# cvlab-kaist/3DGAN-Inversion

Hardware: AMD Instinct MI355X
Metric: inversion-steps/sec (G fwd+bwd, 512^2 FFHQ EG3D) at 1/2/4/8 GPUs; final PSNR (higher is better)
Workload: dtype f32 (modulated convs: two-piece fp16 split, 3 products, range-normalised; other GEMMs bf16x6; fp32-equivalent); 1 GPU; C2: FFHQ 512^2 single-image latent inversion step (Phase A, w + 17 noise maps per image; G.synthesis fwd+bwd, 128^2 x 96-sample rendering, stub-LPIPS feature distance + noise regulariser, Adam); images_per_gpu=1, world_size=1, generator=ffhqrebalanced512-128-shaped, 30.66 M params, random-init (synthetic weights), parallelism=1 independent images, 1 per GPU; stat all-reduce only, launch=one HIP graph replay per step

## Files before the change

3dgan-inversion_amd/csrc/renderer.hip:

```cpp
#include "common.h"
#include "det.h"
#include "render_common.h"

namespace {

constexpr int FC = 32;
constexpr int HD = 64;
constexpr int CO = 32;
#ifndef RK_MAXT
#define RK_MAXT 192
#endif
constexpr int MAXT = RK_MAXT;

__device__ __forceinline__ float sigmoidf_(float x) { return __frcp_rn(1.f + __expf(-x)); }
__device__ __forceinline__ float softplusf_(float x) { return fmaxf(x, 0.f) + __logf(1.f + __expf(-fabsf(x))); }
__device__ __forceinline__ float sigmoid_acc(float x) { return 1.f / (1.f + expf(-x)); }
__device__ __forceinline__ float softplus_acc(float x) { return x > 20.f ? x : log1pf(expf(x)); }

struct PlaneUV { float u, v; };

__device__ __forceinline__ void plane_uv(int pl, float x, float y, float z, float& u, float& v) {
    if (pl == 0) { u = x; v = y; } else if (pl == 1) { u = x; v = z; } else { u = z; v = x; }
}

// ... 519 lines not shown
    float* E = red + r * 2 * D;
    float* GA = red + RPB * 2 * D + r * 2 * D;
    float* GWT = red + 2 * RPB * 2 * D + r * 4 * D;
    float* DL = GWT + 2 * D;
    if (has_c) E[rank_c] = e_c;
    if (has_f) E[rank_f] = e_f;
    __syncthreads();
    float xw[2] = {0.f, 0.f};
    if (live) {
        const float wsum = L.misc[0], dnum = L.misc[1];
        const float depth_raw = dnum / wsum;
        const float dmin = p.depth_minmax[0], dmax = p.depth_minmax[1];
        float gd = bp.d_depth ? bp.d_depth[rr] : 0.f;
        if (!(depth_raw >= dmin && depth_raw <= dmax)) gd = 0.f;
        const float gws = bp.d_wsum ? bp.d_wsum[rr] : 0.f;
        float grgb_sum = 0.f;
        if (p.white_back) for (int k = 0; k < CO; ++k) grgb_sum += grgb[k];
        int k = 0;
        for (int i = s; i < nI; i += D, ++k) {
            const float dmid = 0.5f * (L.sd[i] + L.sd[i + 1]);
            float gw = (E[i] + E[i + 1]) + gws - 2.f * grgb_sum;
            if (gd != 0.f) gw += gd * (dmid - depth_raw) / wsum;
            const float m = 0.5f * (L.ss[i] + L.ss[i + 1]) - 1.f;
            GWT[i] = gw * L.t[i];
            DL[i] = L.sd[i + 1] - L.sd[i];
            GA[i] = m > 20.f ? 1.f : (RK_FAST_ALPHA ? sigmoidf_(m) : sigmoid_acc(m));
            xw[k] = gw * L.w[i];
        }
    }
    __syncthreads();
    if (live) {
        int k = 0;
        for (int i = s; i < nI; i += D, ++k) E[i] = xw[k];
    }
    __syncthreads();
    if (scan_lane) suffix_scan_inplace(red + tid * 2 * D, nI, 2 * D, vec);
    __syncthreads();
    if (live) {
        for (int i = s; i < nI; i += D) {
            const float q = L.q[i];
            const float galpha = GWT[i] - E[i] / q;
            const float one_minus_alpha = q - 1e-10f;
            const float gsp = galpha * DL[i] * one_minus_alpha;
            GA[i] = gsp * GA[i];
        }
    }
    __syncthreads();

    if (bp.df_amax != nullptr && blockIdx.x == 0 && tid == 0) *bp.df_amax = 0.f;
    if (live && s < D) {
        float4* pr = reinterpret_cast<float4*>(bp.df_pos);
        pr[(rr * 2 + 0) * D + s] = has_c ? make_float4(ox + depth_c * dx, oy + depth_c * dy, oz + depth_c * dz, depth_c) : make_float4(NAN, 0, 0, 0);
        pr[(rr * 2 + 1) * D + s] = has_f ? make_float4(ox + depth_f * dx, oy + depth_f * dy, oz + depth_f * dz, depth_f) : make_float4(NAN, 0, 0, 0);
    }
    if (has_c) {
        const float a = 0.5f * ((rank_c > 0 ? L.w[rank_c - 1] : 0.f) + (rank_c < nI ? L.w[rank_c] : 0.f));
        const float gs = 0.5f * ((rank_c > 0 ? GA[rank_c - 1] : 0.f) + (rank_c < nI ? GA[rank_c] : 0.f));
        reinterpret_cast<float2*>(bp.ag_rows)[(rr * 2 + 0) * D + s] = make_float2(a, gs);
    }
    if (has_f) {
        const float a = 0.5f * ((rank_f > 0 ? L.w[rank_f - 1] : 0.f) + (rank_f < nI ? L.w[rank_f] : 0.f));
        const float gs = 0.5f * ((rank_f > 0 ? GA[rank_f - 1] : 0.f) + (rank_f < nI ? GA[rank_f] : 0.f));
        reinterpret_cast<float2*>(bp.ag_rows)[(rr * 2 + 1) * D + s] = make_float2(a, gs);
    }
}

__global__ void __launch_bounds__(256) render_coord_reduce_kernel(const float4* __restrict__ gc, float* __restrict__ d_o, float* __restrict__ d_d,
                                                                  int64_t nrays, int rows_per_ray) {
    const int64_t ray = (int64_t)blockIdx.x * blockDim.x + threadIdx.x;
    if (ray >= nrays) return;
    float o0 = 0.f, o1 = 0.f, o2 = 0.f, d0 = 0.f, d1 = 0.f, d2 = 0.f;
    const float4* g = gc + ray * rows_per_ray;
    for (int i = 0; i < rows_per_ray; ++i) {
        const float4 v = g[i];
        o0 += v.x; o1 += v.y; o2 += v.z;
        d0 += v.x * v.w; d1 += v.y * v.w; d2 += v.z * v.w;
    }
    if (d_o) { d_o[ray * 3] = o0; d_o[ray * 3 + 1] = o1; d_o[ray * 3 + 2] = o2; }
    if (d_d) { d_d[ray * 3] = d0; d_d[ray * 3 + 1] = d1; d_d[ray * 3 + 2] = d2; }
}

constexpr int TS = 15;

__device__ __forceinline__ bool plane_cell(const float4 pos, int pl, float cs, int Hp, int Wp, int& x0, int& y0, float& wx1, float& wy1) {
    float u, v;
    plane_uv(pl, pos.x * cs, pos.y * cs, pos.z * cs, u, v);
    float ix = ((u + 1.f) * Wp - 1.f) * 0.5f, iy = ((v + 1.f) * Hp - 1.f) * 0.5f;
    float fx0 = floorf(ix), fy0 = floorf(iy);
    wx1 = ix - fx0; wy1 = iy - fy0;
    if (!(fx0 >= -1.f && fx0 <= (float)(Wp - 1) && fy0 >= -1.f && fy0 <= (float)(Hp - 1))) return false;
    x0 = (int)fx0; y0 = (int)fy0;
    return true;
}

__device__ __forceinline__ int tile_of(int x0, int y0, int ntx, int nty) {
    int tx = (x0 < 0 ? 0 : x0) / TS, ty = (y0 < 0 ? 0 : y0) / TS;
    return (ty < nty ? ty : nty - 1) * ntx + (tx < ntx ? tx : ntx - 1);
}

constexpr int BIN_ITEMS = 16;
template <int PASS>
__global__ void __launch_bounds__(256) scatter_bin_kernel(const float4* __restrict__ pos, int64_t S, int64_t rows_per_image, float cs, int Hp, int Wp,
                                                          int ntx, int nty, int nb, int* __restrict__ counts, const int* __restrict__ offsets,
                                                          int* __restrict__ fill, int* __restrict__ ids) {
    extern __shared__ int hist[];
    for (int i = threadIdx.x; i < nb; i += 256) hist[i] = 0;
    __syncthreads();
    int bin[BIN_ITEMS], lrank[BIN_ITEMS], rowi[BIN_ITEMS];
    const int64_t base = (int64_t)blockIdx.x * 256 * BIN_ITEMS + threadIdx.x;
#pragma unroll
    for (int k = 0; k < BIN_ITEMS; ++k) {
        bin[k] = -1;
        const int64_t i = base + (int64_t)k * 256;
        if (i >= S * 3) continue;
        const int64_t row = i / 3;
        const int pl = (int)(i - row * 3);
        const float4 ps = pos[row];
        if (isnan(ps.x)) continue;
        int x0, y0; float wx1, wy1;
        if (!plane_cell(ps, pl, cs, Hp, Wp, x0, y0, wx1, wy1)) continue;
        const int n = (int)(row / rows_per_image);
        bin[k] = (n * 3 + pl) * (ntx * nty) + tile_of(x0, y0, ntx, nty);
        rowi[k] = (int)row;
        lrank[k] = atomicAdd(&hist[bin[k]], 1);
    }
    __syncthreads();
    if constexpr (PASS == 0) {
        for (int i = threadIdx.x; i < nb; i += 256) { int c = hist[i]; if (c) atomicAdd(counts + i, c); }
    } else {
        int* basep = hist + nb;
        for (int i = threadIdx.x; i < nb; i += 256) { int c = hist[i]; basep[i] = c ? offsets[i] + atomicAdd(fill + i, c) : 0; }
        __syncthreads();
#pragma unroll
        for (int k = 0; k < BIN_ITEMS; ++k)
            if (bin[k] >= 0) {
                if (PASS == 1) {
                    ids[basep[bin[k]] + lrank[k]] = rowi[k] << 2;
                } else {
                    const int ntile = ntx * nty, t = bin[k] % ntile, pl = (bin[k] / ntile) % 3;
                    int x0, y0; float wx1, wy1;
                    plane_cell(pos[rowi[k]], pl, cs, Hp, Wp, x0, y0, wx1, wy1);
                    const int lx = x0 - (t % ntx) * TS, ly = y0 - (t / ntx) * TS;
                    reinterpret_cast<float4*>(ids)[basep[bin[k]] + lrank[k]] =
                        make_float4(__int_as_float(rowi[k]), __int_as_float(((ly + 1) << 16) | (lx + 1)), wx1, wy1);
                }
            }
    }
}

constexpr int CHUNK = 4096;

__global__ void __launch_bounds__(1024) scatter_scan_kernel(const int* __restrict__ counts, int* __restrict__ offsets, int* __restrict__ chunk_offsets, int n) {
    __shared__ int part[1024], partc[1024];
    const int t = threadIdx.x;
    const int per = (n + 1023) / 1024;
    int sum = 0, sumc = 0;
    for (int k = 0; k < per; ++k) { int idx = t * per + k; if (idx < n) { int c = counts[idx]; sum += c; sumc += (c + CHUNK - 1) / CHUNK; } }
    part[t] = sum; partc[t] = sumc;
    __syncthreads();
    for (int off = 1; off < 1024; off <<= 1) {
        int v = t >= off ? part[t - off] : 0, vc = t >= off ? partc[t - off] : 0;
        __syncthreads();
        part[t] += v; partc[t] += vc;
        __syncthreads();
    }
    int run = part[t] - sum, runc = partc[t] - sumc;
    for (int k = 0; k < per; ++k) {
        int idx = t * per + k;
        if (idx < n) { int c = counts[idx]; offsets[idx] = run; if (chunk_offsets) chunk_offsets[idx] = runc; run += c; runc += (c + CHUNK - 1) / CHUNK; }
    }
// ... 214 lines not shown
    lds_barrier();
    issue_R(0); issue_M(2);
    asm volatile("s_waitcnt vmcnt(3)" ::: "memory");
    lds_barrier();
    issue_R(1);
    for (int b = 0; b < nbat; ++b) {
        asm volatile("s_waitcnt vmcnt(2)" ::: "memory");
        lds_barrier();
        issue_M(b + 3);
        issue_R(b + 2);
        const float4* meta = reinterpret_cast<const float4*>(sm + NRB * ROWB + (b % NMB) * RECB);
        const float* dfb = reinterpret_cast<const float*>(sm + (b % NRB) * ROWB);
        int* cn = cnt[b & 1];
        if (tid < TROWS) cnt[(b + 1) & 1][tid] = 0;
        if (tid < BATCH && beg + b * BATCH + tid < end) {
            const int k = __float_as_int(meta[tid].y) >> 16;
            lists[k * BATCH + lds_add_rtn((unsigned)(uintptr_t)&cn[k], 1)] = (unsigned short)tid;
        }
        lds_barrier();
#pragma unroll
        for (int l = 0; l < LPW; ++l) {
            const int li = wave * LPW + l;
            const int m = cn[li];
            const unsigned short* lst = lists + li * BATCH;
            for (int e = 0; e < m; e += 8) {
                int j[4];
                float4 mt[4];
                float g[4];
#pragma unroll
                for (int q = 0; q < 4; ++q) j[q] = lst[min(e + 2 * q + kk, BATCH - 1)] & (BATCH - 1);
#pragma unroll
                for (int q = 0; q < 4; ++q) { mt[q] = meta[j[q]]; g[q] = dfb[j[q] * FC + c]; }
#pragma unroll
                for (int q = 0; q < 4; ++q) {
                    const bool live = e + 2 * q + kk < m;
                    const int lx = (__float_as_int(mt[q].y) & 0xffff) - 1;
                    const float wx = mx == lx ? 1.f - mt[q].z : (mx == lx + 1 ? mt[q].z : 0.f);
                    const float wy = mhalf ? mt[q].w : 1.f - mt[q].w;
                    acc[l] = __builtin_amdgcn_mfma_f32_32x32x2f32(live ? wx * wy : 0.f, live ? g[q] : 0.f, acc[l], 0, 0, 0);
                }
            }
        }
    }
    asm volatile("s_waitcnt vmcnt(0)" ::: "memory");
    __syncthreads();
#pragma unroll
    for (int l = 0; l < LPW; ++l) {
        const int li = wave * LPW + l;
#pragma unroll
        for (int r = 0; r < 16; ++r) {
            const int m = (r & 3) + 8 * (r >> 2) + 4 * kk;
            if (m >= 16) tile[(li * TROWS + (m & 15)) * FC + c] = acc[l][r];
        }
    }
    __syncthreads();
#pragma unroll
    for (int l = 0; l < LPW; ++l) {
        const int li = wave * LPW + l;
        if (li >= 1) {
#pragma unroll
            for (int r = 0; r < 16; ++r) {
                const int m = (r & 3) + 8 * (r >> 2) + 4 * kk;
                if (m < 16) tile[((li - 1) * TROWS + m) * FC + c] += acc[l][r];
            }
        }
    }
    __syncthreads();
    for (int i = tid; i < TILE_FLOATS; i += NT) {
        const float v = tile[i];
        if (v != 0.f) {
            const int cell = i / FC, ch = i - cell * FC;
            const int yy = ty0 + cell / TROWS, xx = tx0 + cell % TROWS;
            if (yy < Hp && xx < Wp) eg3d_acc(d_planes + (int64_t)n * Hp * Wp * ldp + ((int64_t)yy * Wp + xx) * ldp + pl * FC + ch, v);
        }
    }
}

constexpr int BIN16_THREADS = 1024;
constexpr int BIN16_ITEMS = 18;

template <int PASS, int SL>
__global__ void __launch_bounds__(BIN16_THREADS) scatter_bin16_kernel(const float4* __restrict__ pos, int64_t S, float cs, int Hp, int Wp, int ntx, int nty,
                                                            int nb16, int* __restrict__ counts, const int* __restrict__ offsets, int* __restrict__ fill,
                                                            float4* __restrict__ recs, int ray_w, int rpr) {
    extern __shared__ int hist[];
    for (int i = threadIdx.x; i < nb16; i += BIN16_THREADS) hist[i] = 0;
    __syncthreads();
    int bin[BIN16_ITEMS], lrank[BIN16_ITEMS], rowi[BIN16_ITEMS];
    const int ntile = ntx * nty;
    int brick_row0 = 0;
    if (SL > 0) {
        const int nslab = rpr / SL, slab = blockIdx.x % nslab, pb = blockIdx.x / nslab, ppr = ray_w / 16;
        brick_row0 = ((pb / ppr) * 16 * ray_w + (pb % ppr) * 16) * rpr + slab * SL;
    }
    typedef float b16_f4 __attribute__((ext_vector_type(4)));
    constexpr int BIN16_BATCH = 6;
    static_assert(BIN16_ITEMS % BIN16_BATCH == 0, "batches");
#pragma unroll
    for (int kb = 0; kb < BIN16_ITEMS; kb += BIN16_BATCH) {
        b16_f4 psv[BIN16_BATCH];
        int plv[BIN16_BATCH];
#pragma unroll
        for (int j = 0; j < BIN16_BATCH; ++j) {
            const int k = kb + j;
            bin[k] = -1;
            int64_t row = -1; int pl = 0;
            if (SL > 0) {
                const int u = threadIdx.x + k * BIN16_THREADS;
                if (u < 256 * SL * 3) {
                    pl = u % 3;
                    const int v = u / 3, sidx = v % SL, r = v / SL;
                    row = brick_row0 + ((r >> 4) * ray_w + (r & 15)) * rpr + sidx;
                }
            } else {
                const int64_t i = ((int64_t)blockIdx.x * BIN16_ITEMS + k) * BIN16_THREADS + threadIdx.x;
                if (i < S * 3) { row = i / 3; pl = (int)(i - row * 3); }
            }
            rowi[k] = (int)row;
            plv[j] = pl;
            psv[j] = reinterpret_cast<const b16_f4*>(pos)[row >= 0 ? row : 0];
        }
        asm volatile("" ::: "memory");
#pragma unroll
        for (int j = 0; j < BIN16_BATCH; ++j) {
            const int k = kb + j;
            const float4 ps = make_float4(psv[j].x, psv[j].y, psv[j].z, psv[j].w);
            if (rowi[k] < 0 || isnan(ps.x)) continue;
            int x0, y0; float wx1, wy1;
            if (!plane_cell(ps, plv[j], cs, Hp, Wp, x0, y0, wx1, wy1)) continue;
            const int t = tile_of(x0, y0, ntx, nty);
            bin[k] = (plv[j] * ntile + t) * TROWS + (y0 - (t / ntx) * TS + 1);
            lrank[k] = atomicAdd(&hist[bin[k]], 1);
        }
    }
    __syncthreads();
    if (PASS == 0) {
#pragma unroll
        for (int k = 0; k < BIN16_ITEMS; ++k)
            if (bin[k] >= 0 && lrank[k] == 0) atomicAdd(counts + bin[k], hist[bin[k]]);
        return;
    }
    {
        int got[BIN16_ITEMS], off[BIN16_ITEMS];
#pragma unroll
        for (int k = 0; k < BIN16_ITEMS; ++k) {
            got[k] = 0; off[k] = 0;
            if (bin[k] >= 0 && lrank[k] == 0) { got[k] = atomicAdd(fill + bin[k], hist[bin[k]]); off[k] = offsets[bin[k]]; }
        }
        asm volatile("" ::: "memory");
#pragma unroll
        for (int k = 0; k < BIN16_ITEMS; ++k)
            if (bin[k] >= 0 && lrank[k] == 0) hist[bin[k]] = off[k] + got[k];
    }
    __syncthreads();
#pragma unroll
    for (int kb = 0; kb < BIN16_ITEMS; kb += BIN16_BATCH) {
        b16_f4 psv[BIN16_BATCH];
#pragma unroll
        for (int j = 0; j < BIN16_BATCH; ++j) psv[j] = reinterpret_cast<const b16_f4*>(pos)[bin[kb + j] >= 0 ? rowi[kb + j] : 0];
        asm volatile("" ::: "memory");
#pragma unroll
        for (int j = 0; j < BIN16_BATCH; ++j) {
            const int k = kb + j;
            if (bin[k] >= 0) {
                const int t = (bin[k] / TROWS) % ntile, pl = bin[k] / (TROWS * ntile);
                int x0, y0; float wx1, wy1;
                plane_cell(make_float4(psv[j].x, psv[j].y, psv[j].z, psv[j].w), pl, cs, Hp, Wp, x0, y0, wx1, wy1);
                const int lx = x0 - (t % ntx) * TS;
                recs[hist[bin[k]] + lrank[k]] = make_float4(__int_as_float(rowi[k] | ((lx + 1) << 27)), wx1, wy1, 0.f);
            }
        }
    }
}

__global__ void __launch_bounds__(1024) scatter_scan16_kernel(const int* __restrict__ counts, int* __restrict__ offsets, int n) {
    __shared__ int v[16384 + 512];
    __shared__ int wsum[16];
    const int t = threadIdx.x, lane = t & 63, wave = t >> 6;
    for (int i = t; i < n; i += 1024) v[i + (i >> 5)] = counts[i];
    __syncthreads();
    const int per = (n + 1023) / 1024;
    int sum = 0;
    for (int k = 0; k < per; ++k) { const int i = t * per + k; if (i < n) sum += v[i + (i >> 5)]; }
    int inc = sum;
#pragma unroll
    for (int o = 1; o < 64; o <<= 1) { const int u = __shfl_up(inc, o); if (lane >= o) inc += u; }
    if (lane == 63) wsum[wave] = inc;
    __syncthreads();
    int run = inc - sum;
    for (int w = 0; w < wave; ++w) run += wsum[w];
    for (int k = 0; k < per; ++k) { const int i = t * per + k; if (i < n) { const int c = v[i + (i >> 5)]; v[i + (i >> 5)] = run; run += c; } }
    if (t == 1023) offsets[n] = run;
    __syncthreads();
    for (int i = t; i < n; i += 1024) offsets[i] = v[i + (i >> 5)];
}

#if EG3D_DET
constexpr int SORT16_LDS = 4096;
__global__ void __launch_bounds__(256) scatter_sort16_kernel(const int* __restrict__ offsets, float4* __restrict__ recs) {
    __shared__ __attribute__((aligned(16))) float4 sm[SORT16_LDS];
    const int beg = offsets[blockIdx.x], n = offsets[blockIdx.x + 1] - beg;
    if (n < 2) return;
    float4* g = recs + beg;
    float4* a = n <= SORT16_LDS ? sm : g;
    if (n <= SORT16_LDS) {
        for (int i = threadIdx.x; i < n; i += 256) sm[i] = g[i];
    }
    __syncthreads();
    auto key = [](const float4& r) { return __float_as_int(r.x) & 0x7ffffff; };
    auto cmpx = [&](int i, int l) {
        if (l > i && l < n) {
            const float4 u = a[i], v = a[l];
            if (key(v) < key(u)) { a[i] = v; a[l] = u; }
        }
    };
    for (int k = 2; (k >> 1) < n; k <<= 1) {
        for (int i = threadIdx.x; i < n; i += 256) cmpx(i, i ^ (k - 1));
        __syncthreads();
        for (int j = k >> 2; j > 0; j >>= 1) {
            for (int i = threadIdx.x; i < n; i += 256) cmpx(i, i ^ j);
            __syncthreads();
        }
    }
    if (n <= SORT16_LDS)
        for (int i = threadIdx.x; i < n; i += 256) g[i] = sm[i];
}
#endif

constexpr int ACCP_WAVES = 4;
__global__ void __launch_bounds__(ACCP_WAVES * 64) scatter_accum16p_kernel(const float* __restrict__ df, int64_t S, const int* __restrict__ offsets,
                                                                            const float4* __restrict__ recs, float* __restrict__ d_planes, int Hp, int Wp,
                                                                            int ldp, int ntx, int nty, int split) {
    __shared__ float amat[ACCP_WAVES * 8 * 64];
    __shared__ __attribute__((aligned(16))) float4 recm[ACCP_WAVES * 128];
    __shared__ __attribute__((aligned(16))) int keym[ACCP_WAVES * 128];
    const int tid = threadIdx.x;
    const int ntile = ntx * nty, nlist = 3 * ntile * TROWS;
    const int wave = __builtin_amdgcn_readfirstlane(tid >> 6), lane = tid & 63, c = lane & 31, kk = lane >> 5;
    float* abuf = amat + wave * (8 * 64);
    float4* recl = recm + wave * 128;
    int* keyl = keym + wave * 128;
    for (int i = lane; i < 8 * 64; i += 64) abuf[i] = 0.f;
    const int pj = lane >> 2, half = (lane >> 1) & 1, dx = lane & 1;
    const int a_slot = (pj >> 1) * 64 + (pj & 1) * 32 + half * 16;
    const __amdgpu_buffer_rsrc_t drs = __builtin_amdgcn_make_buffer_rsrc(const_cast<float*>(df), 0, (int)(S * FC * 4), 0x00020000);
    const float4 zero4 = make_float4(0.f, 0.f, 0.f, 0.f);
    const int nwave = gridDim.x * ACCP_WAVES;
    for (int ui = blockIdx.x * ACCP_WAVES + wave; ui < nlist * split; ui += nwave) {
        const int li = ui / split, part = ui - li * split;
        const int lbeg = __builtin_amdgcn_readfirstlane(offsets[li]), llen = __builtin_amdgcn_readfirstlane(offsets[li + 1]) - lbeg;
        const int beg = lbeg + (int)((int64_t)llen * part / split), end = lbeg + (int)((int64_t)llen * (part + 1) / split);
        if (beg >= end) continue;
        acc16_t acc;
#pragma unroll
        for (int i = 0; i < 16; ++i) acc[i] = 0.f;
        auto load_recs = [&](int p0) { return p0 + lane < end ? recs[p0 + lane] : zero4; };
        auto stash = [&](const float4& R, int par) {
            recl[par * 64 + lane] = R;
            keyl[par * 64 + (lane & 48) + (lane & 1) * 8 + ((lane & 15) >> 1)] = __float_as_int(R.x);
        };
        unsigned g[32];
        {
            const float4 R0 = load_recs(beg), R1 = load_recs(beg + 64);
            stash(R0, 0); stash(R1, 1);
        }
#pragma unroll
        for (int gq = 0; gq < 4; ++gq) {
            const int4 k0 = *reinterpret_cast<const int4*>(keyl + gq * 16 + kk * 8), k1 = *reinterpret_cast<const int4*>(keyl + gq * 16 + kk * 8 + 4);
            const int nk[8] = {k0.x, k0.y, k0.z, k0.w, k1.x, k1.y, k1.z, k1.w};
#pragma unroll
            for (int q = 0; q < 8; ++q) g[gq * 8 + q] = __builtin_amdgcn_raw_buffer_load_b32(drs, (nk[q] & 0x7ffffff) * (FC * 4) + c * 4, 0, 0);
        }
        int par = 0;
        for (int p0 = beg; p0 < end; p0 += 64, par ^= 1) {
            const float4 Rnn = load_recs(p0 + 128);
            const int npair = min(64, end - p0);
            const bool more = p0 + 64 < end;
#pragma unroll
            for (int gq = 0; gq < 4; ++gq) {
                if (gq * 16 >= npair && !more) break;
                const float4 R = recl[par * 64 + gq * 16 + pj];
                const int* kp = keyl + (par ^ 1) * 64 + gq * 16 + kk * 8;
                const int4 k0 = *reinterpret_cast<const int4*>(kp), k1 = *reinterpret_cast<const int4*>(kp + 4);
                const int nk[8] = {k0.x, k0.y, k0.z, k0.w, k1.x, k1.y, k1.z, k1.w};
                const int col = (int)((unsigned)__float_as_int(R.x) >> 27) - 1 + dx;
                const float val = (dx ? R.y : 1.f - R.y) * (half ? R.z : 1.f - R.z);
                if (col >= 0) abuf[a_slot + col] = val;
#pragma unroll
                for (int q = 0; q < 8; ++q) {
                    const int Q = gq * 8 + q;
                    acc = __builtin_amdgcn_mfma_f32_32x32x2f32(abuf[q * 64 + lane], __uint_as_float(g[Q]), acc, 0, 0, 0);
                    g[Q] = __builtin_amdgcn_raw_buffer_load_b32(drs, (nk[q] & 0x7ffffff) * (FC * 4) + c * 4, 0, 0);
                }
                if (col >= 0) abuf[a_slot + col] = 0.f;
            }
            stash(Rnn, par);
        }
        const int lrow = li % TROWS, t = (li / TROWS) % ntile, pl = li / (TROWS * ntile);
        const int yy0 = (t / ntx) * TS + lrow - 1, tx0 = (t % ntx) * TS;
        float* base = d_planes + pl * FC + c;
#pragma unroll
        for (int r = 0; r < 16; ++r) {
            const int m = (r & 3) + 8 * (r >> 2) + 4 * kk;
            const int yy = yy0 + (m >> 4), xx = tx0 + (m & 15);
            if (yy >= 0 && yy < Hp && xx < Wp && acc[r] != 0.f) eg3d_acc(base + ((int64_t)yy * Wp + xx) * ldp, acc[r]);
        }
    }
}

typedef _Float16 sc_f16x8 __attribute__((ext_vector_type(8)));
typedef __fp16 sc_fp16x2 __attribute__((ext_vector_type(2)));
__global__ void __launch_bounds__(ACCP_WAVES * 64) scatter_accum16h_kernel(const float* __restrict__ df, int64_t S, const int* __restrict__ offsets,
                                                                            const float4* __restrict__ recs, float* __restrict__ d_planes, int Hp, int Wp,
                                                                            int ldp, int ntx, int nty, const float* __restrict__ df_amax) {
    __shared__ __attribute__((aligned(16))) _Float16 aimg[ACCP_WAVES * 3 * 512];
    __shared__ __attribute__((aligned(16))) float4 recm[ACCP_WAVES * 128];
    __shared__ __attribute__((aligned(16))) int keym[ACCP_WAVES * 128];
    const int tid = threadIdx.x;
    const int ntile = ntx * nty, nlist = 3 * ntile * TROWS;
    const int wave = __builtin_amdgcn_readfirstlane(tid >> 6), lane = tid & 63, c = lane & 31, kk = lane >> 5;
    _Float16* ai = aimg + wave * (3 * 512);
    float4* recl = recm + wave * 128;
    int* keyl = keym + wave * 128;
    for (int i = lane; i < 3 * 512; i += 64) ai[i] = (_Float16)0.f;
    const int pj = lane >> 2, half = (lane >> 1) & 1, dx = lane & 1;
    const int a_slot = half * 16 * 16 + pj;
    const __amdgpu_buffer_rsrc_t drs = __builtin_amdgcn_make_buffer_rsrc(const_cast<float*>(df), 0, (int)(S * FC * 4), 0x00020000);
    const float4 zero4 = make_float4(0.f, 0.f, 0.f, 0.f);
    float sc = 1.f;
    {
        const float am = *df_amax;
        if (am > 0.f && am < 3.0e38f) {
            int e = (int)((__float_as_uint(am) >> 23) & 0xff) - 127;
            e = max(-100, min(100, e));
            sc = __uint_as_float((unsigned)(127 + 13 - e) << 23);
        }
    }
    const float out_mul = 1.f / (sc * 1024.f);
    const int nwave = gridDim.x * ACCP_WAVES;
    for (int li = blockIdx.x * ACCP_WAVES + wave; li < nlist; li += nwave) {
        const int beg = __builtin_amdgcn_readfirstlane(offsets[li]), end = __builtin_amdgcn_readfirstlane(offsets[li + 1]);
        if (beg >= end) continue;
        acc16_t acc;
#pragma unroll
        for (int i = 0; i < 16; ++i) acc[i] = 0.f;
        auto load_recs = [&](int p0) { return p0 + lane < end ? recs[p0 + lane] : zero4; };
        auto stash = [&](const float4& R, int par) { recl[par * 64 + lane] = R; keyl[par * 64 + lane] = __float_as_int(R.x); };
        auto issue_rows = [&](unsigned (&gr)[32], int gq, int par) {
            const int* kp = keyl + par * 64 + gq * 16 + kk * 8;
            const int4 k0 = *reinterpret_cast<const int4*>(kp), k1 = *reinterpret_cast<const int4*>(kp + 4);
            const int nk[8] = {k0.x, k0.y, k0.z, k0.w, k1.x, k1.y, k1.z, k1.w};
#pragma unroll
            for (int j = 0; j < 8; ++j) gr[gq * 8 + j] = __builtin_amdgcn_raw_buffer_load_b32(drs, (nk[j] & 0x7ffffff) * (FC * 4) + c * 4, 0, 0);
        };
        unsigned g[32];
        {
            const float4 R0 = load_recs(beg), R1 = load_recs(beg + 64);
            stash(R0, 0); stash(R1, 1);
        }
#pragma unroll
        for (int gq = 0; gq < 4; ++gq) issue_rows(g, gq, 0);
        int par = 0;
        for (int p0 = beg; p0 < end; p0 += 64, par ^= 1) {
            const float4 Rnn = load_recs(p0 + 128);
            const int npair = min(64, end - p0);
            const bool more = p0 + 64 < end;
#pragma unroll
            for (int gq = 0; gq < 4; ++gq) {
                if (gq * 16 >= npair && !more) break;
                const float4 R = recl[par * 64 + gq * 16 + pj];
                const int col = (int)((unsigned)__float_as_int(R.x) >> 27) - 1 + dx;
                const float w = (dx ? R.y : 1.f - R.y) * (half ? R.z : 1.f - R.z) * 1024.f;
                const sc_fp16x2 hw2 = __builtin_amdgcn_cvt_pkrtz(w, 0.f);
                const _Float16 hw = (_Float16)hw2[0], lw = (_Float16)(w - (float)hw2[0]), gw = hw * (_Float16)0.00048828125f;
                if (col >= 0) { ai[a_slot + col * 16] = hw; ai[512 + a_slot + col * 16] = lw; ai[1024 + a_slot + col * 16] = gw; }
                sc_f16x8 bh, bl;
#pragma unroll
                for (int q = 0; q < 4; ++q) {
                    const float a0 = __uint_as_float(g[gq * 8 + 2 * q]) * sc, a1 = __uint_as_float(g[gq * 8 + 2 * q + 1]) * sc;
                    const sc_fp16x2 hh = __builtin_amdgcn_cvt_pkrtz(a0, a1);
                    bh[2 * q] = (_Float16)hh[0]; bh[2 * q + 1] = (_Float16)hh[1];
                    bl[2 * q] = (_Float16)__builtin_amdgcn_fmed3f((a0 - (float)hh[0]) * 2048.f, -65504.f, 65504.f);
                    bl[2 * q + 1] = (_Float16)__builtin_amdgcn_fmed3f((a1 - (float)hh[1]) * 2048.f, -65504.f, 65504.f);
                }
                issue_rows(g, gq, par ^ 1);
                const sc_f16x8* ap = reinterpret_cast<const sc_f16x8*>(ai) + (lane & 31) * 2 + kk;
                const sc_f16x8 ah = ap[0], al = ap[64], ag = ap[128];
                acc = __builtin_amdgcn_mfma_f32_32x32x16_f16(ag, bl, acc, 0, 0, 0);
                acc = __builtin_amdgcn_mfma_f32_32x32x16_f16(al, bh, acc, 0, 0, 0);
                acc = __builtin_amdgcn_mfma_f32_32x32x16_f16(ah, bh, acc, 0, 0, 0);
                if (col >= 0) { ai[a_slot + col * 16] = (_Float16)0.f; ai[512 + a_slot + col * 16] = (_Float16)0.f; ai[1024 + a_slot + col * 16] = (_Float16)0.f; }
            }
            stash(Rnn, par);
        }
        const int lrow = li % TROWS, t = (li / TROWS) % ntile, pl = li / (TROWS * ntile);
        const int yy0 = (t / ntx) * TS + lrow - 1, tx0 = (t % ntx) * TS;
        float* base = d_planes + pl * FC + c;
#pragma unroll
        for (int r = 0; r < 16; ++r) {
            const int m = (r & 3) + 8 * (r >> 2) + 4 * kk;
            const int yy = yy0 + (m >> 4), xx = tx0 + (m & 15);
            const float v = acc[r] * out_mul;
            if (yy >= 0 && yy < Hp && xx < Wp && v != 0.f) eg3d_acc(base + ((int64_t)yy * Wp + xx) * ldp, v);
        }
    }
}

__global__ void render_finalize_kernel(float* depth, const float* mm, int64_t n) {
    int64_t i = (int64_t)blockIdx.x * blockDim.x + threadIdx.x;
    if (i >= n) return;
    float v = depth[i];
    if (isnan(v)) v = INFINITY;
    if (isinf(v)) v = v > 0 ? 3.4028234663852886e38f : -3.4028234663852886e38f;
    depth[i] = fminf(fmaxf(v, mm[0]), mm[1]);
}

__global__ void __launch_bounds__(256) ray_gen_fwd_kernel(const float* __restrict__ c2w, const float* __restrict__ K, float* __restrict__ origins,
                                                          float* __restrict__ dirs, int N, int res) {
    const int64_t total = (int64_t)N * res * res;
    int64_t i = (int64_t)blockIdx.x * blockDim.x + threadIdx.x;
    if (i >= total) return;
    const int n = (int)(i / (res * res));
    const int pix = (int)(i - (int64_t)n * res * res);
    const int row = pix / res, col = pix - row * res;
    const float* M = c2w + n * 16;
    const float* Kn = K + n * 9;
    const float fx = Kn[0], sk = Kn[1], cx = Kn[2], fy = Kn[4], cy = Kn[5];
    const float inv = (float)(1.0 / res), half = (float)(0.5 / res);
    const float xc = (float)col * inv + half, yc = (float)row * inv + half;
    const float xl = (xc - cx + cy * sk / fy - sk * yc / fy) / fx;
    const float yl = (yc - cy) / fy;
    float v[3];
#pragma unroll
    for (int a = 0; a < 3; ++a) {
        float w = M[a * 4 + 0] * xl + M[a * 4 + 1] * yl + M[a * 4 + 2] + M[a * 4 + 3];
        v[a] = w - M[a * 4 + 3];
        origins[i * 3 + a] = M[a * 4 + 3];
    }
    float nrm = fmaxf(sqrtf(v[0] * v[0] + v[1] * v[1] + v[2] * v[2]), 1e-12f);
    dirs[i * 3 + 0] = v[0] / nrm; dirs[i * 3 + 1] = v[1] / nrm; dirs[i * 3 + 2] = v[2] / nrm;
}

__global__ void __launch_bounds__(256) ray_gen_bwd_kernel(const float* __restrict__ c2w, const float* __restrict__ K, const float* __restrict__ g_o,
                                                          const float* __restrict__ g_d, float* __restrict__ d_c2w, float* __restrict__ d_K, int res) {
    __shared__ float red[4][17];
    const int n = blockIdx.y;
    const float* M = c2w + n * 16;
    const float* Kn = K + n * 9;
    const float fx = Kn[0], sk = Kn[1], cx = Kn[2], fy = Kn[4], cy = Kn[5];
    const float inv = (float)(1.0 / res), half = (float)(0.5 / res);
    float acc[17];
#pragma unroll
    for (int k = 0; k < 17; ++k) acc[k] = 0.f;
    for (int pix = blockIdx.x * blockDim.x + threadIdx.x; pix < res * res; pix += gridDim.x * blockDim.x) {
        const int row = pix / res, col = pix - row * res;
        const int64_t i = (int64_t)n * res * res + pix;
        const float xc = (float)col * inv + half, yc = (float)row * inv + half;
        const float xl = (xc - cx + cy * sk / fy - sk * yc / fy) / fx;
        const float yl = (yc - cy) / fy;
        float v[3], g[3];
#pragma unroll
        for (int a = 0; a < 3; ++a) {
            v[a] = M[a * 4 + 0] * xl + M[a * 4 + 1] * yl + M[a * 4 + 2];
            g[a] = g_d ? g_d[i * 3 + a] : 0.f;
        }
        float nrm = fmaxf(sqrtf(v[0] * v[0] + v[1] * v[1] + v[2] * v[2]), 1e-12f);
        float dn[3] = {v[0] / nrm, v[1] / nrm, v[2] / nrm};
        float dot = dn[0] * g[0] + dn[1] * g[1] + dn[2] * g[2];
        float dxl = 0.f, dyl = 0.f;
#pragma unroll
        for (int a = 0; a < 3; ++a) {
            float dv = (g[a] - dn[a] * dot) / nrm;
            acc[a * 4 + 0] += dv * xl; acc[a * 4 + 1] += dv * yl; acc[a * 4 + 2] += dv;
            acc[a * 4 + 3] += g_o ? g_o[i * 3 + a] : 0.f;
            dxl += dv * M[a * 4 + 0]; dyl += dv * M[a * 4 + 1];
        }
        acc[12] += -xl / fx * dxl;
        acc[13] += (cy / fy - yc / fy) / fx * dxl;
        acc[14] += -dxl / fx;
// ... 80 lines not shown
    hipLaunchKernelGGL(render_kernel<0>, dim3(eg3d_cdiv(nrays, RPB)), dim3(MAXT), render_smem(*pp, 0), st, bp);
    EG3D_LAUNCH_CHECK();
    return EG3D_OK;
}

extern "C" int eg3d_render_finalize(float* depth, const float* depth_minmax, int64_t n, void* stream) {
    if (!depth || !depth_minmax || n < 0) return EG3D_ERR_INVALID;
    if (n == 0) return EG3D_OK;
    hipLaunchKernelGGL(render_finalize_kernel, dim3(eg3d_cdiv(n, 256)), dim3(256), 0, (hipStream_t)stream, depth, depth_minmax, n);
    EG3D_LAUNCH_CHECK();
    return EG3D_OK;
}

extern "C" int eg3d_render_bwd(const eg3d_render_bwd_params* bp, void* stream) {
    if (!bp) return EG3D_ERR_INVALID;
    int rc = check_render(bp->fwd);
    if (rc) return rc;
    const eg3d_render_params& p = bp->fwd;
    if (!bp->d_rgb || !p.depth_minmax || !p.save_sigma || !p.save_rgb || !bp->ag_rows) return EG3D_ERR_INVALID;
    if ((bp->d_origins || bp->d_dirs) && !bp->gc_rows) return EG3D_ERR_INVALID;
    if (!bp->df_pos) return EG3D_ERR_INVALID;
    const int D = p.Dc > p.Df ? p.Dc : p.Df;
    const int RPB = MAXT / D;
    const int64_t nrays = (int64_t)p.N * p.R;
    hipStream_t st = (hipStream_t)stream;
    hipLaunchKernelGGL(render_kernel<1>, dim3(eg3d_cdiv(nrays, RPB)), dim3(MAXT), render_smem(p, 1), st, *bp);
    const int64_t S = nrays * 2 * D;
    EG3D_DET_SCOPE(det, stream);
    EG3D_DET_BIND(det, bp->gram_w0, HD * FC); EG3D_DET_BIND(det, bp->gram_b0, HD); EG3D_DET_BIND(det, bp->gram_w1, (1 + CO) * HD); EG3D_DET_BIND(det, bp->gram_b1, 1 + CO);
    EG3D_DET_COMMIT(det);
    if (int rc2 = eg3d_decode_rows_bwd(*bp, bp->df_pos, 0, S, (int64_t)p.R * 2 * D, 2 * D, stream)) return rc2;
    EG3D_DET_END(det);
    if (bp->d_origins || bp->d_dirs)
        hipLaunchKernelGGL(render_coord_reduce_kernel, dim3(eg3d_cdiv(nrays, 256)), dim3(256), 0, st, reinterpret_cast<const float4*>(bp->gc_rows),
                           bp->d_origins, bp->d_dirs, nrays, 2 * D);
    EG3D_LAUNCH_CHECK();
    return EG3D_OK;
}

extern "C" int eg3d_render_query_sizes(const eg3d_render_params* p, eg3d_render_sizes* out) {
    if (!p || !out || p->N <= 0 || p->R <= 0 || p->Dc <= 0 || p->Df < 0 || p->Cout <= 0) return EG3D_ERR_INVALID;
    const int64_t NR = (int64_t)p->N * p->R, D = p->Dc > p->Df ? p->Dc : p->Df, S = NR * 2 * D;
    out->S = S;
    out->rgb = NR * p->Cout;  out->depth = NR;  out->wsum = NR;  out->depth_minmax = 2;
    out->fine_depths = NR * p->Df;
    out->save_sigma = S;  out->save_rgb = S * p->Cout;  out->pos_rows = p->Df > 0 ? 2 * NR * D * 4 : 0;
    out->df_rows = S * FC;  out->df_pos = S * 4;  out->ag_rows = S * 2;  out->gc_rows = S * 4;
    out->dump_dpre = S * 64;  out->dump_h = S * 64;  out->dump_dout = S * (1 + p->Cout);  out->dump_feat = S * FC;
    out->feat_rows = p->Df > 0 ? S * FC : 0;
    return EG3D_OK;
}

extern "C" int64_t eg3d_triplane_scatter_workspace_ints(int64_t S, int N, int Hp, int Wp) {
    const int64_t nb = (int64_t)N * 3 * ((Hp + TS - 1) / TS) * ((Wp + TS - 1) / TS);
    const int64_t nb16 = 3 * ((Hp + TS - 1) / TS) * ((Wp + TS - 1) / TS) * (TS + 1);
    return (4 * nb + 2 > 3 * nb16 + 2 ? 4 * nb + 2 : 3 * nb16 + 2) + 3 + 12 * S;
}

extern "C" int eg3d_triplane_scatter(const float* df_rows, const float* df_pos, int64_t S, int64_t rows_per_image, float* d_planes, int N, int Hp,
                                     int Wp, int ldp, float box_warp, int32_t* workspace, int ray_w, int rows_per_ray, const float* df_amax, void* stream) {
    if (!df_rows || !df_pos || !d_planes || !workspace || S <= 0 || N <= 0 || rows_per_image <= 0) return EG3D_ERR_INVALID;
    if (ldp < 3 * FC || 3 * S > INT32_MAX / 4) return EG3D_ERR_UNSUPPORTED;
    const int ntx = (Wp + TS - 1) / TS, nty = (Hp + TS - 1) / TS;
    const int nb = N * 3 * ntx * nty;
    if ((size_t)nb * 2 * sizeof(int) > 64 * 1024) return EG3D_ERR_UNSUPPORTED;
    int* counts = workspace;
    int* fill = counts + nb;
    int* offsets = fill + nb;
    int* chunk_offsets = offsets + nb + 1;
    int* ids = chunk_offsets + nb + 1;
    ids += (4 - ((ids - workspace) & 3)) & 3;
    hipStream_t st = (hipStream_t)stream;
    const float cs = 2.f / box_warp;
    EG3D_DET_SCOPE(det, stream); EG3D_DET_BIND(det, d_planes, (int64_t)N * Hp * Wp * ldp); EG3D_DET_COMMIT(det);
    const int blocks = eg3d_cdiv(S * 3, 256 * BIN_ITEMS);
    const float4* pos4 = reinterpret_cast<const float4*>(df_pos);
    static const int variant0 = [] { const char* e = getenv("EG3D_SCATTER"); return e ? atoi(e) : 4; }();
    const int nb16_img = 3 * ntx * nty * TROWS;
    if (variant0 == 4 && nb16_img <= 16384 && S % N == 0 && rows_per_image == S / N && rows_per_image * FC * 4 < ((int64_t)1 << 32)
        && rows_per_image < (1 << 27)) {
        int* counts16 = workspace;
        int* fill16 = counts16 + nb16_img;
        int* offsets16 = fill16 + nb16_img;
        int* recs_i = offsets16 + nb16_img + 1;
        recs_i += (4 - ((recs_i - workspace) & 3)) & 3;
        float4* recs = reinterpret_cast<float4*>(recs_i);
        const int64_t Si = rows_per_image;
        int SL = 0;
        if (ray_w > 0 && rows_per_ray > 0 && ray_w % 16 == 0 && Si % ((int64_t)rows_per_ray * ray_w) == 0 && (Si / ((int64_t)rows_per_ray * ray_w)) % 16 == 0)
            SL = rows_per_ray % 24 == 0 ? 24 : (rows_per_ray % 16 == 0 ? 16 : 0);
        const int blocks_i = SL ? (int)(Si / rows_per_ray / 256 * (rows_per_ray / SL)) : eg3d_cdiv(Si * 3, BIN16_THREADS * BIN16_ITEMS);
        auto bin_pass = [&](int pass, const float4* pos_n) {
#define EG3D_BIN16(P, L) hipLaunchKernelGGL((scatter_bin16_kernel<P, L>), dim3(blocks_i), dim3(BIN16_THREADS), sizeof(int) * nb16_img, st, pos_n, Si, cs, Hp, \
                                            Wp, ntx, nty, nb16_img, counts16, offsets16, fill16, recs, ray_w, rows_per_ray)
            if (pass == 0) { if (SL == 24) EG3D_BIN16(0, 24); else if (SL == 16) EG3D_BIN16(0, 16); else EG3D_BIN16(0, 0); }
            else           { if (SL == 24) EG3D_BIN16(1, 24); else if (SL == 16) EG3D_BIN16(1, 16); else EG3D_BIN16(1, 0); }
#undef EG3D_BIN16
        };
        for (int n = 0; n < N; ++n) {
            const float4* pos_n = pos4 + (int64_t)n * Si;
            eg3d_zero_words(counts16, 2 * (int64_t)nb16_img, st);
            bin_pass(0, pos_n);
            hipLaunchKernelGGL(scatter_scan16_kernel, dim3(1), dim3(1024), 0, st, counts16, offsets16, nb16_img);
            bin_pass(1, pos_n);
#if EG3D_DET
            hipLaunchKernelGGL(scatter_sort16_kernel, dim3(nb16_img), dim3(256), 0, st, offsets16, recs);
#endif
            constexpr int split = 1;
            const int accb = (nb16_img + ACCP_WAVES - 1) / ACCP_WAVES;
            if (df_amax != nullptr) {
                hipLaunchKernelGGL(scatter_accum16h_kernel, dim3(accb), dim3(ACCP_WAVES * 64), 0, st, df_rows + (int64_t)n * Si * FC, Si, offsets16, recs,
                                   d_planes + (int64_t)n * Hp * Wp * ldp, Hp, Wp, ldp, ntx, nty, df_amax);
                continue;
            }
            hipLaunchKernelGGL(scatter_accum16p_kernel, dim3(accb), dim3(ACCP_WAVES * 64), 0, st, df_rows + (int64_t)n * Si * FC, Si, offsets16, recs,
                               d_planes + (int64_t)n * Hp * Wp * ldp, Hp, Wp, ldp, ntx, nty, split);
        }
        EG3D_DET_END(det);
        EG3D_LAUNCH_CHECK();
        return EG3D_OK;
    }
#if EG3D_DET
    return EG3D_ERR_UNSUPPORTED;
#endif
    eg3d_zero_words(counts, 2 * (int64_t)nb, st);
    hipLaunchKernelGGL(scatter_bin_kernel<0>, dim3(blocks), dim3(256), sizeof(int) * nb, st, pos4, S, rows_per_image, cs, Hp, Wp, ntx, nty, nb, counts,
                       offsets, fill, ids);
    hipLaunchKernelGGL(scatter_scan_kernel, dim3(1), dim3(1024), 0, st, counts, offsets, chunk_offsets, nb);
    const int max_chunks = (int)((3 * S + CHUNK - 1) / CHUNK) + nb;
    const int variant = variant0 == 4 ? 3 : variant0;
    if (variant == 1 || S * FC * 4 >= ((int64_t)1 << 32) || 3 * S * 16 >= ((int64_t)1 << 32)) {
        hipLaunchKernelGGL(scatter_bin_kernel<1>, dim3(blocks), dim3(256), sizeof(int) * 2 * nb, st, pos4, S, rows_per_image, cs, Hp, Wp, ntx, nty, nb, counts,
                           offsets, fill, ids);
        hipLaunchKernelGGL(scatter_accum_kernel, dim3(max_chunks), dim3(ACC_THREADS), 0, st, df_rows, pos4, offsets, chunk_offsets, ids, d_planes, cs, Hp, Wp, ldp,
                           ntx, nty, nb);
    } else {
        hipLaunchKernelGGL(scatter_bin_kernel<2>, dim3(blocks), dim3(256), sizeof(int) * 2 * nb, st, pos4, S, rows_per_image, cs, Hp, Wp, ntx, nty, nb, counts,
                           offsets, fill, ids);
        const float4* recs = reinterpret_cast<const float4*>(ids);
        hipLaunchKernelGGL((scatter_accum2_kernel<16, 256>), dim3(max_chunks), dim3(1024), 0, st, df_rows, S, offsets, chunk_offsets, recs, 3 * S, d_planes, Hp, Wp,
                           ldp, ntx, nty, nb);
    }
    EG3D_LAUNCH_CHECK();
    return EG3D_OK;
}

extern "C" int eg3d_sample_decode(const eg3d_render_params* pp, const float* coords, int64_t M, float* rgb, float* sigma, void* stream) {
    if (!pp || !coords || !rgb || !sigma || M < 0) return EG3D_ERR_INVALID;
    const eg3d_render_params& p = *pp;
    if (!p.planes || !p.w0 || !p.b0 || !p.w1 || !p.b1 || p.N <= 0) return EG3D_ERR_INVALID;
    if (p.C != FC || p.Hdim != HD || p.Cout != CO || p.ldp < 3 * FC || (p.ldp & 3)) return EG3D_ERR_UNSUPPORTED;
    if (M == 0) return EG3D_OK;
    eg3d_render_params q = p;
    q.feat_rows = nullptr;
    return eg3d_decode_rows_fwd(q, coords, 3, (int64_t)p.N * M, M, sigma, rgb, stream);
}

extern "C" int eg3d_ray_gen_fwd(const float* cam2world, const float* intrinsics, float* origins, float* dirs, int N, int res, void* stream) {
    if (!cam2world || !intrinsics || !origins || !dirs || N <= 0 || res <= 0) return EG3D_ERR_INVALID;
    hipLaunchKernelGGL(ray_gen_fwd_kernel, dim3(eg3d_cdiv((int64_t)N * res * res, 256)), dim3(256), 0, (hipStream_t)stream, cam2world, intrinsics,
                       origins, dirs, N, res);
    EG3D_LAUNCH_CHECK();
    return EG3D_OK;
}

extern "C" int eg3d_ray_gen_bwd(const float* cam2world, const float* intrinsics, const float* d_origins, const float* d_dirs, float* d_cam2world,
                                float* d_intrinsics, int N, int res, void* stream) {
    if (!cam2world || !intrinsics || !d_cam2world || N <= 0 || res <= 0) return EG3D_ERR_INVALID;
    hipStream_t st = (hipStream_t)stream;
    eg3d_zero_words(d_cam2world, 16 * (int64_t)N, st);
    if (d_intrinsics) eg3d_zero_words(d_intrinsics, 9 * (int64_t)N, st);
    int bx = std::min(eg3d_cdiv((int64_t)res * res, 256), 64);
    EG3D_DET_SCOPE(det, stream); EG3D_DET_BIND(det, d_cam2world, 16 * (int64_t)N); EG3D_DET_BIND(det, d_intrinsics, 9 * (int64_t)N); EG3D_DET_COMMIT(det);
    hipLaunchKernelGGL(ray_gen_bwd_kernel, dim3(bx, N), dim3(256), 0, st, cam2world, intrinsics, d_origins, d_dirs, d_cam2world, d_intrinsics, res);
    EG3D_DET_END(det);
    EG3D_LAUNCH_CHECK();
    return EG3D_OK;
}
```

Measured before the change: 232.5 steps/s.

## Shrink scatter-bin records to packed int keys; recompute weights in accumulate

The binning pass now stores only a 4-byte packed key (row index plus local x offset) per sample instead of a 16-byte float4 record with bilinear weights. It also drops the second position reload and plane_cell evaluation from the bin kernel's write phase. The accumulate kernels instead gather each sample's position through a buffer load and recompute the fractional weights from the tile origin, with key and position prefetch pipelined one and two batches ahead. The deterministic sort kernel now sorts ints, so it can hold four times as many entries in LDS. The trade is less record write/read traffic in exchange for an extra indirect gather of positions in the accumulate loop.

```diff
diff --git a/3dgan-inversion_amd/csrc/renderer.hip b/3dgan-inversion_amd/csrc/renderer.hip
--- a/3dgan-inversion_amd/csrc/renderer.hip
+++ b/3dgan-inversion_amd/csrc/renderer.hip
@@ -625,10 +625,15 @@
 
 constexpr int TS = 15;
 
-__device__ __forceinline__ bool plane_cell(const float4 pos, int pl, float cs, int Hp, int Wp, int& x0, int& y0, float& wx1, float& wy1) {
+__device__ __forceinline__ void plane_ixy(const float4 pos, int pl, float cs, int Hp, int Wp, float& ix, float& iy) {
     float u, v;
     plane_uv(pl, pos.x * cs, pos.y * cs, pos.z * cs, u, v);
-    float ix = ((u + 1.f) * Wp - 1.f) * 0.5f, iy = ((v + 1.f) * Hp - 1.f) * 0.5f;
+    ix = ((u + 1.f) * Wp - 1.f) * 0.5f; iy = ((v + 1.f) * Hp - 1.f) * 0.5f;
+}
+
+__device__ __forceinline__ bool plane_cell(const float4 pos, int pl, float cs, int Hp, int Wp, int& x0, int& y0, float& wx1, float& wy1) {
+    float ix, iy;
+    plane_ixy(pos, pl, cs, Hp, Wp, ix, iy);
     float fx0 = floorf(ix), fy0 = floorf(iy);
     wx1 = ix - fx0; wy1 = iy - fy0;
     if (!(fx0 >= -1.f && fx0 <= (float)(Wp - 1) && fy0 >= -1.f && fy0 <= (float)(Hp - 1))) return false;
@@ -1009,7 +1014,7 @@
 template <int PASS, int SL>
 __global__ void __launch_bounds__(BIN16_THREADS) scatter_bin16_kernel(const float4* __restrict__ pos, int64_t S, float cs, int Hp, int Wp, int ntx, int nty,
                                                             int nb16, int* __restrict__ counts, const int* __restrict__ offsets, int* __restrict__ fill,
-                                                            float4* __restrict__ recs, int ray_w, int rpr) {
+                                                            int* __restrict__ recs, int ray_w, int rpr) {
     extern __shared__ int hist[];
     for (int i = threadIdx.x; i < nb16; i += BIN16_THREADS) hist[i] = 0;
     __syncthreads();
@@ -1057,6 +1062,7 @@
             if (!plane_cell(ps, plv[j], cs, Hp, Wp, x0, y0, wx1, wy1)) continue;
             const int t = tile_of(x0, y0, ntx, nty);
             bin[k] = (plv[j] * ntile + t) * TROWS + (y0 - (t / ntx) * TS + 1);
+            if (PASS == 1) rowi[k] |= (x0 - (t % ntx) * TS + 1) << 27;
             lrank[k] = atomicAdd(&hist[bin[k]], 1);
         }
     }
@@ -1081,23 +1087,8 @@
     }
     __syncthreads();
 #pragma unroll
-    for (int kb = 0; kb < BIN16_ITEMS; kb += BIN16_BATCH) {
-        b16_f4 psv[BIN16_BATCH];
-#pragma unroll
-        for (int j = 0; j < BIN16_BATCH; ++j) psv[j] = reinterpret_cast<const b16_f4*>(pos)[bin[kb + j] >= 0 ? rowi[kb + j] : 0];
-        asm volatile("" ::: "memory");
-#pragma unroll
-        for (int j = 0; j < BIN16_BATCH; ++j) {
-            const int k = kb + j;
-            if (bin[k] >= 0) {
-                const int t = (bin[k] / TROWS) % ntile, pl = bin[k] / (TROWS * ntile);
-                int x0, y0; float wx1, wy1;
-                plane_cell(make_float4(psv[j].x, psv[j].y, psv[j].z, psv[j].w), pl, cs, Hp, Wp, x0, y0, wx1, wy1);
-                const int lx = x0 - (t % ntx) * TS;
-                recs[hist[bin[k]] + lrank[k]] = make_float4(__int_as_float(rowi[k] | ((lx + 1) << 27)), wx1, wy1, 0.f);
-            }
-        }
-    }
+    for (int k = 0; k < BIN16_ITEMS; ++k)
+        if (bin[k] >= 0) recs[hist[bin[k]] + lrank[k]] = rowi[k];
 }
 
 __global__ void __launch_bounds__(1024) scatter_scan16_kernel(const int* __restrict__ counts, int* __restrict__ offsets, int n) {
@@ -1123,21 +1114,21 @@
 }
 
 #if EG3D_DET
-constexpr int SORT16_LDS = 4096;
-__global__ void __launch_bounds__(256) scatter_sort16_kernel(const int* __restrict__ offsets, float4* __restrict__ recs) {
-    __shared__ __attribute__((aligned(16))) float4 sm[SORT16_LDS];
+constexpr int SORT16_LDS = 16384;
+__global__ void __launch_bounds__(256) scatter_sort16_kernel(const int* __restrict__ offsets, int* __restrict__ recs) {
+    __shared__ int sm[SORT16_LDS];
     const int beg = offsets[blockIdx.x], n = offsets[blockIdx.x + 1] - beg;
     if (n < 2) return;
-    float4* g = recs + beg;
-    float4* a = n <= SORT16_LDS ? sm : g;
+    int* g = recs + beg;
+    int* a = n <= SORT16_LDS ? sm : g;
     if (n <= SORT16_LDS) {
         for (int i = threadIdx.x; i < n; i += 256) sm[i] = g[i];
     }
     __syncthreads();
-    auto key = [](const float4& r) { return __float_as_int(r.x) & 0x7ffffff; };
+    auto key = [](int r) { return r & 0x7ffffff; };
     auto cmpx = [&](int i, int l) {
         if (l > i && l < n) {
-            const float4 u = a[i], v = a[l];
+            const int u = a[i], v = a[l];
             if (key(v) < key(u)) { a[i] = v; a[l] = u; }
         }
     };
@@ -1155,9 +1146,10 @@
 #endif
 
 constexpr int ACCP_WAVES = 4;
-__global__ void __launch_bounds__(ACCP_WAVES * 64) scatter_accum16p_kernel(const float* __restrict__ df, int64_t S, const int* __restrict__ offsets,
-                                                                            const float4* __restrict__ recs, float* __restrict__ d_planes, int Hp, int Wp,
-                                                                            int ldp, int ntx, int nty, int split) {
+typedef unsigned sc_u32x4 __attribute__((ext_vector_type(4)));
+__global__ void __launch_bounds__(ACCP_WAVES * 64) scatter_accum16p_kernel(const float* __restrict__ df, const float4* __restrict__ pos, int64_t S, float cs,
+                                                                            const int* __restrict__ offsets, const int* __restrict__ recs,
+                                                                            float* __restrict__ d_planes, int Hp, int Wp, int ldp, int ntx, int nty, int split) {
     __shared__ float amat[ACCP_WAVES * 8 * 64];
     __shared__ __attribute__((aligned(16))) float4 recm[ACCP_WAVES * 128];
     __shared__ __attribute__((aligned(16))) int keym[ACCP_WAVES * 128];
@@ -1171,7 +1163,7 @@
     const int pj = lane >> 2, half = (lane >> 1) & 1, dx = lane & 1;
     const int a_slot = (pj >> 1) * 64 + (pj & 1) * 32 + half * 16;
     const __amdgpu_buffer_rsrc_t drs = __builtin_amdgcn_make_buffer_rsrc(const_cast<float*>(df), 0, (int)(S * FC * 4), 0x00020000);
-    const float4 zero4 = make_float4(0.f, 0.f, 0.f, 0.f);
+    const __amdgpu_buffer_rsrc_t prs = __builtin_amdgcn_make_buffer_rsrc(const_cast<float4*>(pos), 0, (int)(S * 16), 0x00020000);
     const int nwave = gridDim.x * ACCP_WAVES;
     for (int ui = blockIdx.x * ACCP_WAVES + wave; ui < nlist * split; ui += nwave) {
         const int li = ui / split, part = ui - li * split;
@@ -1181,15 +1173,27 @@
         acc16_t acc;
 #pragma unroll
         for (int i = 0; i < 16; ++i) acc[i] = 0.f;
-        auto load_recs = [&](int p0) { return p0 + lane < end ? recs[p0 + lane] : zero4; };
+        const int lrow = li % TROWS, t = (li / TROWS) % ntile, pl = li / (TROWS * ntile);
+        const int yy0 = (t / ntx) * TS + lrow - 1, tx0 = (t % ntx) * TS;
+        const float fy0 = (float)yy0;
+        auto load_keys = [&](int p0) { return p0 + lane < end ? recs[p0 + lane] : 0; };
+        auto load_pos = [&](int key) { return __builtin_amdgcn_raw_buffer_load_b128(prs, (key & 0x7ffffff) * 16, 0, 0); };
+        auto make_rec = [&](int key, const sc_u32x4& P, int p0) {
+            float ix, iy;
+            plane_ixy(make_float4(__uint_as_float(P.x), __uint_as_float(P.y), __uint_as_float(P.z), __uint_as_float(P.w)), pl, cs, Hp, Wp, ix, iy);
+            const bool valid = p0 + lane < end;
+            const float fx0 = (float)(tx0 + (int)((unsigned)key >> 27) - 1);
+            return make_float4(__int_as_float(key), valid ? ix - fx0 : 0.f, valid ? iy - fy0 : 0.f, 0.f);
+        };
         auto stash = [&](const float4& R, int par) {
             recl[par * 64 + lane] = R;
             keyl[par * 64 + (lane & 48) + (lane & 1) * 8 + ((lane & 15) >> 1)] = __float_as_int(R.x);
         };
         unsigned g[32];
         {
-            const float4 R0 = load_recs(beg), R1 = load_recs(beg + 64);
-            stash(R0, 0); stash(R1, 1);
+            const int K0 = load_keys(beg), K1 = load_keys(beg + 64);
+            const sc_u32x4 P0 = load_pos(K0), P1 = load_pos(K1);
+            stash(make_rec(K0, P0, beg), 0); stash(make_rec(K1, P1, beg + 64), 1);
         }
 #pragma unroll
         for (int gq = 0; gq < 4; ++gq) {
@@ -1198,9 +1202,11 @@
 #pragma unroll
             for (int q = 0; q < 8; ++q) g[gq * 8 + q] = __builtin_amdgcn_raw_buffer_load_b32(drs, (nk[q] & 0x7ffffff) * (FC * 4) + c * 4, 0, 0);
         }
+        int Kn = load_keys(beg + 128);
         int par = 0;
         for (int p0 = beg; p0 < end; p0 += 64, par ^= 1) {
-            const float4 Rnn = load_recs(p0 + 128);
+            const sc_u32x4 Pnn = load_pos(Kn);
+            const int Knn = load_keys(p0 + 192);
             const int npair = min(64, end - p0);
             const bool more = p0 + 64 < end;
 #pragma unroll
@@ -1221,10 +1227,9 @@
                 }
                 if (col >= 0) abuf[a_slot + col] = 0.f;
             }
-            stash(Rnn, par);
-        }
-        const int lrow = li % TROWS, t = (li / TROWS) % ntile, pl = li / (TROWS * ntile);
-        const int yy0 = (t / ntx) * TS + lrow - 1, tx0 = (t % ntx) * TS;
+            stash(make_rec(Kn, Pnn, p0 + 128), par);
+            Kn = Knn;
+        }
         float* base = d_planes + pl * FC + c;
 #pragma unroll
         for (int r = 0; r < 16; ++r) {
@@ -1237,9 +1242,10 @@
 
 typedef _Float16 sc_f16x8 __attribute__((ext_vector_type(8)));
 typedef __fp16 sc_fp16x2 __attribute__((ext_vector_type(2)));
-__global__ void __launch_bounds__(ACCP_WAVES * 64) scatter_accum16h_kernel(const float* __restrict__ df, int64_t S, const int* __restrict__ offsets,
-                                                                            const float4* __restrict__ recs, float* __restrict__ d_planes, int Hp, int Wp,
-                                                                            int ldp, int ntx, int nty, const float* __restrict__ df_amax) {
+__global__ void __launch_bounds__(ACCP_WAVES * 64) scatter_accum16h_kernel(const float* __restrict__ df, const float4* __restrict__ pos, int64_t S, float cs,
+                                                                            const int* __restrict__ offsets, const int* __restrict__ recs,
+                                                                            float* __restrict__ d_planes, int Hp, int Wp, int ldp, int ntx, int nty,
+                                                                            const float* __restrict__ df_amax) {
     __shared__ __attribute__((aligned(16))) _Float16 aimg[ACCP_WAVES * 3 * 512];
     __shared__ __attribute__((aligned(16))) float4 recm[ACCP_WAVES * 128];
     __shared__ __attribute__((aligned(16))) int keym[ACCP_WAVES * 128];
@@ -1253,7 +1259,7 @@
     const int pj = lane >> 2, half = (lane >> 1) & 1, dx = lane & 1;
     const int a_slot = half * 16 * 16 + pj;
     const __amdgpu_buffer_rsrc_t drs = __builtin_amdgcn_make_buffer_rsrc(const_cast<float*>(df), 0, (int)(S * FC * 4), 0x00020000);
-    const float4 zero4 = make_float4(0.f, 0.f, 0.f, 0.f);
+    const __amdgpu_buffer_rsrc_t prs = __builtin_amdgcn_make_buffer_rsrc(const_cast<float4*>(pos), 0, (int)(S * 16), 0x00020000);
     float sc = 1.f;
     {
         const float am = *df_amax;
@@ -1271,7 +1277,18 @@
         acc16_t acc;
 #pragma unroll
         for (int i = 0; i < 16; ++i) acc[i] = 0.f;
-        auto load_recs = [&](int p0) { return p0 + lane < end ? recs[p0 + lane] : zero4; };
+        const int lrow = li % TROWS, t = (li / TROWS) % ntile, pl = li / (TROWS * ntile);
+        const int yy0 = (t / ntx) * TS + lrow - 1, tx0 = (t % ntx) * TS;
+        const float fy0 = (float)yy0;
+        auto load_keys = [&](int p0) { return p0 + lane < end ? recs[p0 + lane] : 0; };
+        auto load_pos = [&](int key) { return __builtin_amdgcn_raw_buffer_load_b128(prs, (key & 0x7ffffff) * 16, 0, 0); };
+        auto make_rec = [&](int key, const sc_u32x4& P, int p0) {
+            float ix, iy;
+            plane_ixy(make_float4(__uint_as_float(P.x), __uint_as_float(P.y), __uint_as_float(P.z), __uint_as_float(P.w)), pl, cs, Hp, Wp, ix, iy);
+            const bool valid = p0 + lane < end;
+            const float fx0 = (float)(tx0 + (int)((unsigned)key >> 27) - 1);
+            return make_float4(__int_as_float(key), valid ? ix - fx0 : 0.f, valid ? iy - fy0 : 0.f, 0.f);
+        };
         auto stash = [&](const float4& R, int par) { recl[par * 64 + lane] = R; keyl[par * 64 + lane] = __float_as_int(R.x); };
         auto issue_rows = [&](unsigned (&gr)[32], int gq, int par) {
             const int* kp = keyl + par * 64 + gq * 16 + kk * 8;
@@ -1282,14 +1299,17 @@
         };
         unsigned g[32];
         {
-            const float4 R0 = load_recs(beg), R1 = load_recs(beg + 64);
-            stash(R0, 0); stash(R1, 1);
+            const int K0 = load_keys(beg), K1 = load_keys(beg + 64);
+            const sc_u32x4 P0 = load_pos(K0), P1 = load_pos(K1);
+            stash(make_rec(K0, P0, beg), 0); stash(make_rec(K1, P1, beg + 64), 1);
         }
 #pragma unroll
         for (int gq = 0; gq < 4; ++gq) issue_rows(g, gq, 0);
+        int Kn = load_keys(beg + 128);
         int par = 0;
         for (int p0 = beg; p0 < end; p0 += 64, par ^= 1) {
-            const float4 Rnn = load_recs(p0 + 128);
+            const sc_u32x4 Pnn = load_pos(Kn);
+            const int Knn = load_keys(p0 + 192);
             const int npair = min(64, end - p0);
             const bool more = p0 + 64 < end;
 #pragma unroll
@@ -1318,10 +1338,9 @@
                 acc = __builtin_amdgcn_mfma_f32_32x32x16_f16(ah, bh, acc, 0, 0, 0);
                 if (col >= 0) { ai[a_slot + col * 16] = (_Float16)0.f; ai[512 + a_slot + col * 16] = (_Float16)0.f; ai[1024 + a_slot + col * 16] = (_Float16)0.f; }
             }
-            stash(Rnn, par);
-        }
-        const int lrow = li % TROWS, t = (li / TROWS) % ntile, pl = li / (TROWS * ntile);
-        const int yy0 = (t / ntx) * TS + lrow - 1, tx0 = (t % ntx) * TS;
+            stash(make_rec(Kn, Pnn, p0 + 128), par);
+            Kn = Knn;
+        }
         float* base = d_planes + pl * FC + c;
 #pragma unroll
         for (int r = 0; r < 16; ++r) {
@@ -1568,9 +1587,8 @@
         int* counts16 = workspace;
         int* fill16 = counts16 + nb16_img;
         int* offsets16 = fill16 + nb16_img;
-        int* recs_i = offsets16 + nb16_img + 1;
-        recs_i += (4 - ((recs_i - workspace) & 3)) & 3;
-        float4* recs = reinterpret_cast<float4*>(recs_i);
+        int* recs = offsets16 + nb16_img + 1;
+        recs += (4 - ((recs - workspace) & 3)) & 3;
         const int64_t Si = rows_per_image;
         int SL = 0;
         if (ray_w > 0 && rows_per_ray > 0 && ray_w % 16 == 0 && Si % ((int64_t)rows_per_ray * ray_w) == 0 && (Si / ((int64_t)rows_per_ray * ray_w)) % 16 == 0)
@@ -1595,12 +1613,12 @@
             constexpr int split = 1;
             const int accb = (nb16_img + ACCP_WAVES - 1) / ACCP_WAVES;
             if (df_amax != nullptr) {
-                hipLaunchKernelGGL(scatter_accum16h_kernel, dim3(accb), dim3(ACCP_WAVES * 64), 0, st, df_rows + (int64_t)n * Si * FC, Si, offsets16, recs,
-                                   d_planes + (int64_t)n * Hp * Wp * ldp, Hp, Wp, ldp, ntx, nty, df_amax);
+                hipLaunchKernelGGL(scatter_accum16h_kernel, dim3(accb), dim3(ACCP_WAVES * 64), 0, st, df_rows + (int64_t)n * Si * FC, pos_n, Si, cs, offsets16,
+                                   recs, d_planes + (int64_t)n * Hp * Wp * ldp, Hp, Wp, ldp, ntx, nty, df_amax);
                 continue;
             }
-            hipLaunchKernelGGL(scatter_accum16p_kernel, dim3(accb), dim3(ACCP_WAVES * 64), 0, st, df_rows + (int64_t)n * Si * FC, Si, offsets16, recs,
-                               d_planes + (int64_t)n * Hp * Wp * ldp, Hp, Wp, ldp, ntx, nty, split);
+            hipLaunchKernelGGL(scatter_accum16p_kernel, dim3(accb), dim3(ACCP_WAVES * 64), 0, st, df_rows + (int64_t)n * Si * FC, pos_n, Si, cs, offsets16,
+                               recs, d_planes + (int64_t)n * Hp * Wp * ldp, Hp, Wp, ldp, ntx, nty, split);
         }
         EG3D_DET_END(det);
         EG3D_LAUNCH_CHECK();
```

Result: no change. 231.4 steps/s (-0.5%).
